# Gnnng/SVDFeature

Measured on AMD Instinct MI355X. Metric: training instances/sec (SGD updates/s), basicMF k=64, higher is better.
Workload: dtype f32; 1 GPU; basicMF synthetic 1000000x100000, 100000000 ratings, k=64 fp32 (BASELINE configs[1]); order=uniform random (file order preserved: result == sequential SGD), conflict_free_batches_per_pass=903, parallelism=1 GPU

## Files before the change

### svdfeature_amd/csrc/svdf_capi.cpp

```cpp
#include <svdfeature_amd.h>

#include <algorithm>
#include <cstdlib>
#include <cstring>
#include <new>
#include <vector>

#include "svdf_engine.h"
#include "svdf_kernels.h"

namespace svdf {
void rank_eval_metrics(long S, const int64_t *sec_ptr, const int *position, const int *ranked, const int *nan, int num_at, const int *at,
                       svdf_rank_metrics *out);
void set_error_mode(int m);
const char *last_error();
void note_error(const std::string &m);
}

struct svdf_trainer { svdf::Engine *e; };
struct svdf_dataset { svdf::Dataset *d; };
struct svdf_ranker { svdf::Ranker *r; };

#define SVDF_GUARD(retval, ...)                                 \
    try { __VA_ARGS__; }                                        \
// ... 219 lines not shown
    delete ds;
}
int svdf_train_dataset(svdf_trainer *t, svdf_dataset *ds) { SVDF_GUARD(-1, { t->e->train_dataset(ds->d); return 0; }) }
int svdf_predict_dataset(svdf_trainer *t, svdf_dataset *ds, float *out) { SVDF_GUARD(-1, { t->e->predict_dataset(ds->d, out); return 0; }) }
int64_t svdf_dataset_info(const svdf_dataset *ds, int what) {
    if (!ds || !ds->d) return -1;
    switch (what) {
    case 0: return ds->d->num_row;
    case 1: return ds->d->kind == 8 ? (int64_t)ds->d->wchild.size() : (int64_t)ds->d->sched.num_levels();
    case 2: return ds->d->sched.max_level_size;
    case 3: return ds->d->kind;
    case 4: return ds->d->algorithmic_bytes;
    case 5: return ds->d->num_units;
    case 6: return ds->d->num_simple_units;
    case 7: {
        uint64_t h = 1469598103934665603ull;
        auto mix = [&h](uint64_t v) { for (int b = 0; b < 8; b++) { h ^= (v >> (8 * b)) & 0xFFu; h *= 1099511628211ull; } };
        for (long v : ds->d->sched.level_ptr) mix((uint64_t)v);
        for (long v : ds->d->sched.level_mid) mix((uint64_t)v);
        for (int v : ds->d->sched.order) mix((uint64_t)(unsigned)v);
        return (int64_t)(h >> 1);
    }
    case 8: return ds->d->kind == 8 && !ds->d->wchild.empty() ? (int64_t)ds->d->wchild[0]->kind : -1;
    default: return -1;
    }
}

int svdf_item_delta_begin(svdf_trainer *t) { SVDF_GUARD(-1, { t->e->per_rank_api(); t->e->item_delta_begin(); return 0; }) }
void *svdf_item_delta_buffer(svdf_trainer *t, int64_t *count) { SVDF_GUARD(nullptr, { t->e->per_rank_api(); return t->e->item_delta_buffer(count); }) }
int svdf_item_delta_apply(svdf_trainer *t) { SVDF_GUARD(-1, { t->e->per_rank_api(); t->e->item_delta_apply(); return 0; }) }
int svdf_item_delta_export(svdf_trainer *t, float *dst) { SVDF_GUARD(-1, { t->e->per_rank_api(); t->e->item_delta_copy(dst, nullptr); return 0; }) }
int svdf_item_delta_import(svdf_trainer *t, const float *src) { SVDF_GUARD(-1, { t->e->per_rank_api(); t->e->item_delta_copy(nullptr, src); return 0; }) }

int svdf_item_delta_into(svdf_trainer *t, float *dst, int64_t *count) { SVDF_GUARD(-1, { t->e->per_rank_api(); t->e->item_delta_into(dst, count); return 0; }) }
int svdf_item_delta_pack(svdf_trainer *t, void *dst, int half, int64_t *count) { SVDF_GUARD(-1, { t->e->per_rank_api(); t->e->item_delta_pack(dst, half, count); return 0; }) }
int svdf_item_delta_unpack(svdf_trainer *t, const void *src, int half, int refresh_snapshot) {
    SVDF_GUARD(-1, { t->e->per_rank_api(); t->e->item_delta_unpack(src, half, refresh_snapshot); return 0; })
}
int svdf_item_delta_select(svdf_trainer *t, int part, int nparts) { SVDF_GUARD(-1, { t->e->per_rank_api(); t->e->item_delta_select(part, nparts); return 0; }) }
int svdf_item_delta_apply_from(svdf_trainer *t, const float *src) { SVDF_GUARD(-1, { t->e->per_rank_api(); t->e->item_delta_apply_from(src); return 0; }) }
int svdf_set_stream(svdf_trainer *t, void *hip_stream) { SVDF_GUARD(-1, { t->e->set_stream((hipStream_t)hip_stream); return 0; }) }

int64_t svdf_get_view(svdf_trainer *t, int which, float *out, int64_t capacity) { SVDF_GUARD(-1, { return t->e->get_view(which, out, capacity); }) }
int64_t svdf_set_view(svdf_trainer *t, int which, const float *in, int64_t count) { SVDF_GUARD(-1, { return t->e->set_view(which, in, count); }) }
int svdf_view_shape(svdf_trainer *t, int which, int *rows, int *cols) { SVDF_GUARD(-1, { t->e->view_shape(which, rows, cols); return 0; }) }
void *svdf_stream(svdf_trainer *t) { return (void *)t->e->stream(); }
// ... 91 lines not shown
```

### svdfeature_amd/csrc/svdf_config.cpp

```cpp
#include "svdf_engine.h"

#include <algorithm>
#include <chrono>
#include <cmath>
#include <cstdlib>
#include <cstring>
#include <memory>
#include <mutex>
#include <atomic>
#include <thread>

#include "svdf_kernels.h"
#include "svdf_internal.h"

namespace svdf {

void ParamSet::set_param(const char *name, const char *val) {
    if (!strncmp(name, prefix_a.c_str(), prefix_a.size())) name += prefix_a.size();
    else if (!strncmp(name, prefix_b.c_str(), prefix_b.size())) name += prefix_b.size();
    else return;
    if (!strcmp("bound", name)) {
        unsigned bd = (unsigned)atoi(val);
        check(bd > 0, "can't give 0 as bound");
        check(bound.empty() || bound.back() < bd, "bound must be given in order");
// ... 195 lines not shown
        check(value >= 0 && value <= 8 && value != 7, "groups_per_wave must be 0 (auto), 1 ... 6 or 8");
        groups_per_wave_ = (int)value;
        return 0;
    }
    if (!strcmp(name, "xcd_remap")) { xcd_remap_ = value != 0; params_dirty_ = true; return 0; }
    if (!strcmp(name, "fewrow_i16")) { check(value >= 0 && value <= 1, "fewrow_i16 must be 0 or 1"); fewrow_i16_ = (int)value; params_dirty_ = true; return 0; }
    if (!strcmp(name, "svdpp_helpers")) { check(value == 1 || value == 4 || value == 8 || value == 16, "svdpp_helpers must be 1, 4, 8 or 16"); svdpp_helpers_ = (int)value; params_dirty_ = true; return 0; }
    if (!strcmp(name, "basic_i8")) { check(value >= 0 && value <= 1, "basic_i8 must be 0 or 1"); basic_i8_ = (int)value; params_dirty_ = true; return 0; }
    if (!strcmp(name, "load_mode")) { check(value >= 0 && value <= 2, "load_mode must be 0, 1 or 2 (auto)"); load_mode_ = (int)value; params_dirty_ = true; return 0; }
    if (!strcmp(name, "store_mode")) { check(value >= 0 && value <= 2, "store_mode must be 0, 1 or 2"); store_mode_ = (int)value; params_dirty_ = true; return 0; }
    if (!strcmp(name, "sort_batches")) { check(value >= 0 && value <= 2, "sort_batches must be 0, 1 (by item) or 2 (by user)"); sort_batches_ = (int)value; return 0; }
    if (!strcmp(name, "async_flush")) { flush(); async_flush_ = value != 0; return 0; }
    if (!strcmp(name, "use_fused")) { use_fused_ = value != 0; return 0; }
    if (!strcmp(name, "device_schedule")) { device_sched_ = value != 0; return 0; }
    if (!strcmp(name, "device_rank")) { device_rank_ = value != 0; return 0; }
    if (!strcmp(name, "device_init")) { device_init_ = value != 0; return 0; }
    if (!strcmp(name, "device_window")) { device_window_ = value != 0; return 0; }
    if (!strcmp(name, "device_load")) { device_load_ = value != 0; return 0; }
    if (!strcmp(name, "runs_exec")) { check(value == 0 || value == 1, "runs_exec must be 0 or 1"); runs_exec_ = (int)value; return 0; }
    if (!strcmp(name, "runs_len")) { check(value >= 2 && value <= 7, "runs_len must be in 2 .. 7"); runs_len_ = (int)value; return 0; }
    if (!strcmp(name, "runs_sets")) { check(value >= 1 && value <= 2, "runs_sets must be 1 or 2"); runs_sets_ = (int)value; return 0; }
    if (!strcmp(name, "runs_block")) { check(value == 64 || value == 128 || value == 256, "runs_block must be 64, 128 or 256"); runs_block_ = (int)value; return 0; }
    if (!strcmp(name, "runs_min_rows")) { check(value >= 0, "runs_min_rows must not be negative"); runs_min_rows_ = value; return 0; }
    if (!strcmp(name, "pair_units")) { check(value == 0 || value == 1, "pair_units must be 0 or 1"); pair_units_ = (int)value; return 0; }
    if (!strcmp(name, "pair_unit_cap")) { check(value >= 1 && value <= 4096, "pair_unit_cap must be in 1 .. 4096"); pair_unit_cap_ = (int)value; return 0; }
    if (!strcmp(name, "pivot_exec")) { check(value == 0 || value == 1, "pivot_exec must be 0 or 1"); pivot_exec_ = (int)value; return 0; }
    if (!strcmp(name, "pivot_run")) { check(value >= 1 && value <= 65536, "pivot_run must be in 1 .. 65536"); pivot_run_ = (int)value; return 0; }
    if (!strcmp(name, "pivot_min")) { check(value >= 2, "pivot_min must be at least 2"); pivot_min_ = (int)value; return 0; }
    if (!strcmp(name, "ipc_spin_limit")) { ipc_set_spin_limit(value); return 0; }
    if (!strcmp(name, "chain_width")) { check(value >= 0, "chain_width must not be negative"); chain_width_ = value; return 0; }
    if (!strcmp(name, "device_init_margin_log2")) { check(value >= 8 && value <= 52, "device_init_margin_log2 must be in 8 .. 52"); device_init_margin_log2_ = (int)value; return 0; }
    if (!strcmp(name, "device_schedule_min")) { check(value >= 1, "device_schedule_min must be >= 1"); device_sched_min_ = value; return 0; }
    if (!strcmp(name, "use_simple_units")) { use_simple_units_ = value != 0; return 0; }
    if (!strcmp(name, "rows_without_feedback")) { rows_without_feedback_ = value != 0; return 0; }
    if (!strcmp(name, "fewrow_gslots")) { fewrow_gslots_ = value != 0; launch_version_++; return 0; }
    if (!strcmp(name, "staged_pool")) { check(value == 0 || value == 1, "staged_pool must be 0 or 1"); flush(); staged_pool_mode_ = (int)value; return 0; }
    if (!strcmp(name, "wunit_inplace")) { wunit_inplace_ = value != 0; return 0; }
    if (!strcmp(name, "wunit_defer_fb")) { wunit_defer_fb_ = value != 0; return 0; }
    if (!strcmp(name, "wunit_fast")) { check(value >= 0 && value <= 3, "wunit_fast must be 0, 1, 2 or 3"); wunit_fast_ = (int)value; return 0; }
    if (!strcmp(name, "window_per_target_child")) { check(value >= 1, "window_per_target_child must be positive"); wseq_per_target_child_ = (int)value; return 0; }
    if (!strcmp(name, "window_per_target_shared")) { check(value >= 1, "window_per_target_shared must be positive"); wseq_per_target_shared_ = (int)value; return 0; }
    if (!strcmp(name, "window_per_target_fb")) { check(value >= 1, "window_per_target_fb must be positive"); wseq_per_target_fb_ = (int)value; return 0; }
    if (!strcmp(name, "window_shared_sub")) { check(value >= 0 && value <= 4096, "window_shared_sub must be in 0 .. 4096"); wseq_shared_sub_ = (int)value; return 0; }
    if (!strcmp(name, "window_shared_max")) { check(value >= 1, "window_shared_max must be positive"); wseq_shared_max_ = (int)value; return 0; }
    if (!strcmp(name, "window_item_sub")) { check(value >= 0 && value <= 128, "window_item_sub must be in 0 .. 128"); wseq_item_sub_ = (int)value; return 0; }
    if (!strcmp(name, "window_item_max")) { check(value >= 1, "window_item_max must be positive"); wseq_item_max_ = (int)value; return 0; }
// ... 43 lines not shown
```

### svdfeature_amd/csrc/svdf_dataset.cpp

```cpp
#include "svdf_engine.h"

#include <algorithm>
#include <chrono>
#include <cmath>
#include <cstdlib>
#include <cstring>
#include <memory>
#include <mutex>
#include <atomic>
#include <thread>

#include "svdf_kernels.h"
#include "svdf_internal.h"

namespace svdf {

Dataset *Engine::dataset_from_blocks(long num_block, const int *extend_tag, const int64_t *fb_ptr, const unsigned *fb_index, const float *fb_value,
                                     const int64_t *block_row_ptr, const float *row_label, const int64_t *row_ptr, const unsigned *feat_index,
                                     const float *feat_value) {
    check(trainer_ready_, "dataset: init_trainer has not been called");
    need_device("dataset");
    check(user_group(), "svdfeature_amd: block datasets are for user-group (format_type 1) trainers");
    if (multi_ && !in_multi_scope()) {
        check(mp_.common_feedback_space == 0, "svdfeature_amd: amd:gpus > 1 needs a feedback space of its own (common_feedback_space = 0)");
// ... 568 lines not shown
    auto levels = [&](const char *what) { snprintf(buf, sizeof(buf), "exact, %ld conflict-free levels: %s", L, what); return std::string(buf); };
    switch (ds->kind) {
    case 0: return levels(chain_width_ > 0 ? "contract kernel k_basicmf / k_basicmf_slots, one (user, item) instance per lane group; narrow levels chained (k_basicmf_slots_chain)"
                                           : "contract kernel k_basicmf / k_basicmf_slots, one (user, item) instance per lane group");
    case 1: return levels("general sparse kernel k_general (any number of ids per row, side tables, lazy decay)");
    case 2: {
        const FusedSchedule S = ds->fused.view();
        if (fewrow_gslots_ && fewrow_fast_ && fewrow_gslots_applies(P, S, ds->fused.max_nu, ds->fused.max_ni, ds->fused.dense_slots))
            return levels("few-row kernel with global ids k_fewrow_gslots (neighbourhood shape)");
        return levels(fewrow_fast_ && fewrow_fast_applies(P, S) ? "few-row kernel k_fewrow_slots (<= 2 user + 2 item rows per instance: rank pairs, side ids); narrow levels chained"
                                                                 : "fused few-row kernel k_fused");
    }
    case 3: snprintf(buf, sizeof(buf), "exact, %ld conflict-free levels of user units: k_svdpp_wave (one wave per user, %ld of %ld units) + k_svdpp (general units)",
                     L, ds->num_simple_units, ds->num_units); return buf;
    case 4: return levels("multi-level implicit feedback units k_imfb");
    case 5: return "window data set (one window of the window-minibatch step, user side exact): k_window_users / k_window_items";
    case 6: return "amd:gpus handle: per-rank windows (svdf_multi.cpp)";
    case 7: return "window data set of user units: k_wunit_* (svdf_k_wunit.hip)";
    case 8: snprintf(buf, sizeof(buf), "window sequence (amd:step = minibatch / auto): %zu windows, each trained and applied in place%s%s; NOT the reference's sequential semantics (|dRMSE| <= 1e-4 contract)",
                     ds->wchild.size(), side_tables() ? ", feature_user / feature_item children as shared rows (general walk k_wunit_walk)" : "",
                     !ds->wchild.empty() && ds->wchild[0]->kind == 7 && !wunit_width_ok() ? ", user units of wide rows: the wide general walk k_wunit_walk<64, ., ., WideRow>, one wave per unit" : ""); return buf;
    case 9: snprintf(buf, sizeof(buf), "exact, %ld levels: hot rows walked as units (k_svdpp_wave on %s parameters, %ld units) + cold ratings through the contract kernel",
                     L, ds->pv_item_pivot ? "transposed" : "plain", ds->num_units); return buf;
    case 10: snprintf(buf, sizeof(buf), "exact, %ld levels of runs: k_basicmf_runs_soa (up to %d consecutive ratings of one item per lane group, the item's row in registers)", L, ds->rn_len); return buf;
    case 11: snprintf(buf, sizeof(buf), "exact, %ld levels of user-run units: k_pair_units (%ld units of up to %d consecutive pairs of one user, the user's row in registers)",
                      L, ds->num_units, pair_unit_cap_); return buf;
    default: return "unknown";
    }
}
void Engine::note_dataset(Dataset *ds) {
    if (!ds || host_only_ || is_peer_) return;
    const bool verbose = getenv("SVDF_VERBOSE") != nullptr, quiet = getenv("SVDF_QUIET") != nullptr;
    if (verbose && !quiet) fprintf(stderr, "[svdfeature_amd] data set of %ld rows -> %s\n", (long)ds->num_row, path_for(ds).c_str());
    if (step_auto_set_ || step_minibatch_set_ || multi_ || gpus_ != 1) return;
    if (!(ds->kind == 0 || ds->kind == 1 || ds->kind == 2 || ds->kind == 3 || ds->kind == 4 || ds->kind == 9 || ds->kind == 10 || ds->kind == 11) || ds->num_row <= 0) return;
    AutoDecision D;
    double unit_us = 4.5;
    auto_measures(ds, D.levels, unit_us, D.dag_ms, D.stream_ms, pivot_run_);
    guard_last_ = D;
    if (D.dag_ms <= 10.0 * D.stream_ms || D.dag_ms < 50.0) return;
    n_guard_warnings_++;
    if (quiet) return;
    const bool window_ok = ds->plain_rows ? wunit_config_ok(false) && window_rows_allowed() && (wseq_pair_sub_ == 0 || wunit_width_ok())
                                          : wunit_config_ok() && (ds->kind == 3 || ds->kind == 4 || basic_fast_path_allowed());
    fprintf(stderr, "[svdfeature_amd] default (exact) step: %ld rows in %ld conflict-free levels -- the data's dependency depth binds: about %.0f ms per pass "
                    "(%.2f M rows/s; levels x %.1f us) against %.1f ms if the rows streamed.  The exact pass keeps the reference's sequential result bit for bit; "
                    "%s\n",
// ... 235 lines not shown
```

### svdfeature_amd/csrc/svdf_engine.h

```cpp
#ifndef SVDF_ENGINE_H_
#define SVDF_ENGINE_H_

#include <hip/hip_runtime.h>

#include <condition_variable>
#include <cstdio>
#include <memory>
#include <mutex>
#include <stdexcept>
#include <thread>
#include <string>
#include <deque>
#include <functional>
#include <future>
#include <map>
#include <vector>

#include "svdf_types.h"

namespace svdf {

struct Error : std::runtime_error {
    explicit Error(const std::string &m) : std::runtime_error(m) {}
};
// ... 204 lines not shown
    size_t scan_tmp_bytes = 0;
    ~RankSource() { if (scan_tmp) (void)hipFree(scan_tmp); }
};
class Engine;
class Ranker;

struct Dataset {
    Engine *owner = nullptr;
    long num_row = 0;
    int kind = 0;
    DevBuf<WinUser> win_urec;
    DevBuf<int> win_slot, win_iptr, win_slot1;
    DevBuf<unsigned> win_item1;
    DevBuf<float> win_ival1;
    long win_item_lo = 0, win_item_hi = -1;
    DevBuf<long> d_level_ptr;
    bool d_level_ptr_ok = false;
    DevBuf<PairUnit> pu_units;
    DevBuf<unsigned> pu_lo, pu_hi;
    DevBuf<float> pu_vlo, pu_one;
    DevBuf<unsigned> rn_item, rn_user[8];
    DevBuf<float> rn_label[8];
    int rn_len = 0;
    std::vector<long> pv_unit_ptr;
    bool pv_item_pivot = false;
    long pv_cold = 0, pv_hot_rows = 0;
    int64_t chained_levels = 0;
    bool win_hot = false;
    long win_slots = 0;
    DevBuf<int> win_pos;
    bool win_has_pos = false;
    std::vector<long> wfirst;
    DevBuf<WinUnit> wu_units;
    DevBuf<WinSeg> wu_segs;
    DevBuf<int> wu_rptr, wu_tptr, wu_gptr;
    DevBuf<WinEnt> wu_ent, wu_fbent;
    DevBuf<WinTouched> wu_touched;
    long wu_ntouched = -1;
    DevBuf<WinFbRec> wu_fbrec;
    long wu_nseg = 0;
    bool wu_defer_fb = false;
    long wu_gslots = 0;
    int wu_estride = 0;
    bool wu_feedback = false;
    DevBuf<int> wu_uptr, wu_upos;
    DevBuf<WinEnt> wu_uent;
// ... 377 lines not shown
    long wseq_actual_csr(long W, long n, const int64_t *row_ptr, const unsigned *feat_index, const WseqCounts &C0, int shared_sub, int item_sub) const;
    bool wseq_hot_ok() const;
    long wseq_windows_hot(long n, const std::vector<long> &item_count) const;
    long wseq_windows_sub(long n, const std::vector<long> &item_count, int sub, int cap) const;
    void wseq_pair_check(const char *what) const;
    void wseq_sub_check(const char *what, const char *knob, const char *desc, const char *entry, const char *nrank, bool entry_only = false) const;
    std::vector<long> wseq_item_counts(long n, const unsigned *item, const unsigned *item1) const;
    Dataset *wseq_from_columns(long n, const unsigned *user, const unsigned *item, const unsigned *item1, const float *label, int sub, long W);
    double wseq_class_term(const std::vector<long> &cnt, int per) const;
    void wseq_count_targets(WseqCounts &C, long r0, long r1, const int64_t *row_ptr, const unsigned *feat_index) const;
    void wseq_adopt_window(Dataset *ds, const WUnitHost &H, long first);
    long wseq_windows_shared(long n, const std::vector<long> &plain, const std::vector<long> &child, int sub, int cap, int per_plain, int per_child) const;
    double wseq_max_ratio() const { return (double)wseq_per_target_ / (double)wseq_per_target_max_; }
    int wseq_per_target_ = 24;
    bool single_minibatch() const { return step_minibatch_set_ && gpus_ == 1 && !multi_ && !is_peer_; }
    int runs_exec_ = 1;
    int runs_len_ = 4;
    int runs_sets_ = 1, runs_block_ = 64;
    long runs_min_rows_ = 1 << 20;
    int64_t n_runs_passes_ = 0;
    bool runs_config_ok() const;
    Dataset *runs_dataset_from_triples(long n, const unsigned *user, const unsigned *item, const float *label);
    void runs_train(Dataset *ds);
    int pivot_exec_ = 1;
    int pivot_run_ = 256, pivot_run_long_ = 256;
    int pivot_min_ = 2048;
    int64_t n_pivot_passes_ = 0;
    int pair_units_ = 1, pair_unit_cap_ = 16;
    int64_t n_punit_passes_ = 0;
    bool punit_config_ok() const;
    Dataset *punit_dataset_from_pairs(long n, const unsigned *user, const unsigned *pos, const unsigned *neg);
    bool punit_build(long n, const unsigned *user, const unsigned *lo, const unsigned *hi, std::vector<PairUnit> &sorted, std::vector<long> &level_ptr) const;
    bool punit_flush(HostCSR &src);
    DevBuf<PairUnit> w_pu_units_;
    PairUnitSchedule punit_view(const Dataset *ds) const;
    void punit_train(Dataset *ds);
    void punit_predict(Dataset *ds, float *d_out);
    bool pivot_config_ok() const;
    Dataset *pivot_dataset_from_triples(long n, const unsigned *user, const unsigned *item, const float *label);
    void pivot_train(Dataset *ds);
    bool step_auto_set_ = false, auto_building_ = false;
    struct AutoDecision { int decided = 0; long levels = 0, windows = 0; double dag_ms = 0.0, stream_ms = 0.0; } auto_last_;
    bool auto_step_active() const { return step_auto_set_ && !auto_building_ && gpus_ == 1 && !multi_ && !is_peer_ && !host_only_; }
    Dataset *auto_step(Dataset *exact, bool window_ok, const std::function<Dataset *()> &build_window);
    static constexpr long AUTO_PROBE_ROWS = 2000000, AUTO_PROBE_MIN = 8000000;
    AutoDecision auto_probe_;
// ... 186 lines not shown
```

### svdfeature_amd/csrc/svdf_k_runs.hip

```cpp
#include "svdf_device.h"

namespace svdf {

__global__ __launch_bounds__(256) void k_runs_check(const unsigned *user, const unsigned *item, long n, unsigned nu, unsigned ni, unsigned *flag) {
    const long stride = (long)gridDim.x * blockDim.x;
    unsigned bad = 0u;
    for (long p = (long)blockIdx.x * blockDim.x + threadIdx.x; p < n; p += stride) {
        if (user[p] >= nu) bad |= 1u;
        if (item[p] >= ni) bad |= 2u;
    }
    if (bad) atomicOr(flag, bad);
}
__global__ __launch_bounds__(256) void k_runs_prev(const unsigned *keys, const unsigned *pos, long n, unsigned *prev) {
    const long stride = (long)gridDim.x * blockDim.x;
    for (long j = (long)blockIdx.x * blockDim.x + threadIdx.x; j < n; j += stride)
        prev[pos[j]] = (j > 0 && keys[j - 1] == keys[j]) ? pos[j - 1] : 0xFFFFFFFFu;
}
__global__ __launch_bounds__(256) void k_runs_form(const unsigned *ikeys, const unsigned *ipos, long n, unsigned num_item, const unsigned *prev, int R,
                                                   unsigned *head, unsigned *head_of, unsigned char *idx) {
    const long stride = (long)gridDim.x * blockDim.x;
    for (long it = (long)blockIdx.x * blockDim.x + threadIdx.x; it < (long)num_item; it += stride) {
        long lo = 0, hi = n;
        while (lo < hi) { const long mid = (lo + hi) >> 1; if (ikeys[mid] < (unsigned)it) lo = mid + 1; else hi = mid; }
        unsigned h = 0u;
// ... 35 lines not shown
}
void launch_runs_form(const unsigned *ikeys, const unsigned *ipos, long n, unsigned num_item, const unsigned *prev, int R, unsigned *head, unsigned *head_of,
                      unsigned char *idx, hipStream_t st) {
    if (n > 0 && num_item > 0) hipLaunchKernelGGL(k_runs_form, dim3(runs_grid((long)num_item)), dim3(256), 0, st, ikeys, ipos, n, num_item, prev, R, head, head_of, idx);
}
void launch_runs_fill(const unsigned *user, const unsigned *item, const float *label, long n, const unsigned *unit_at, const unsigned *head_of,
                      const unsigned char *idx, long nunit, unsigned *c_item, unsigned *c_user, float *c_label, hipStream_t st) {
    if (n > 0) hipLaunchKernelGGL(k_runs_fill, dim3(runs_grid(n)), dim3(256), 0, st, user, item, label, n, unit_at, head_of, idx, nunit, c_item, c_user, c_label);
}
__global__ __launch_bounds__(256) void k_runs_iota(unsigned *v, long n) {
    const long stride = (long)gridDim.x * blockDim.x;
    for (long j = (long)blockIdx.x * blockDim.x + threadIdx.x; j < n; j += stride) v[j] = (unsigned)j;
}
void launch_runs_iota(unsigned *v, long n, hipStream_t st) {
    if (n <= 0) return;
    long grid = (n + 255) / 256;
    if (grid > 16384) grid = 16384;
    hipLaunchKernelGGL(k_runs_iota, dim3((int)grid), dim3(256), 0, st, v, n);
}
void launch_runs_fill_u32(unsigned *v, long n, unsigned x, hipStream_t st) {
    if (n > 0) hipLaunchKernelGGL(k_runs_fill_u32, dim3(runs_grid(n)), dim3(256), 0, st, v, n, x);
}

template <int LANES, int V, int R, int G>
__global__ __launch_bounds__(256) void k_basicmf_runs_soa(const DevParams P, const RunSchedule S, long begin, long end) {
    constexpr int T = 16 / LANES;
    constexpr int IPS = 64 / LANES;
    constexpr int K = 4 * LANES * V;
    const int lane = threadIdx.x & 63;
    long tile = blockIdx.x;
    if (P.xcd_remap) tile = (long)(blockIdx.x & 7) * (gridDim.x >> 3) + (blockIdx.x >> 3);
    const long wave = tile * (blockDim.x >> 6) + (threadIdx.x >> 6);
    const int m = (lane & 15) / T;
    const int gslot = (lane >> 4) * T + (lane & (T - 1));
    const int pitch = P.pitch;
    const float dec_u1 = snap_to_one(1.0f - P.lr * P.wd_user), dec_i1 = snap_to_one(1.0f - P.lr * P.wd_item);
#pragma unroll 1
    for (int g = 0; g < G; g++) {
        const long w0 = begin + (wave * G + g) * IPS;
        if (w0 >= end) return;
        const long s = w0 + gslot;
        const bool live = s < end;
        const long sc = live ? s : w0;
        const unsigned ir = P.item_off + S.item[sc];
        unsigned ur[R];
        float label[R], bu[R];
        float4 p[R][V], q[V];
        int n = 0;
#pragma unroll
        for (int j = 0; j < R; j++) {
            const unsigned u = S.user[j][sc];
            label[j] = S.label[j][sc];
            const bool on = live && u != (unsigned)SLOT_ABSENT;
            ur[j] = P.user_off + (on ? u : 0u);
            if (on) n = j + 1;
        }
#pragma unroll
        for (int v = 0; v < V; v++) q[v] = live ? load_row_nt<K / 4>(P.W, ir, pitch, m + v * LANES, K) : f4zero();
        float bi = live ? P.bias[ir] : 0.0f;
#pragma unroll
        for (int j = 0; j < R; j++) {
#pragma unroll
            for (int v = 0; v < V; v++) p[j][v] = f4zero();
            bu[j] = 0.0f;
            if (j < n) {
#pragma unroll
                for (int v = 0; v < V; v++) p[j][v] = load_row_nt<K / 4>(P.W, ur[j], pitch, m + v * LANES, K);
                bu[j] = P.bias[ur[j]];
            }
        }
#pragma unroll
        for (int j = 0; j < R; j++) asm volatile("" :: "v"(p[j][0].x), "v"(p[j][V - 1].x), "v"(bu[j]));
#pragma unroll
        for (int j = 0; j < R; j++) {
            if (!__any(j < n)) break;
            double bs = 0.0;
            bs += (double)(1.0f * bu[j]); bs += 0.0;
            bs += 0.0;
            bs += (double)(1.0f * bi);
            double sum = (double)P.base_score + bs;
            float4 tu[V], ti[V];
#pragma unroll
            for (int v = 0; v < V; v++) { tu[v] = f4zero(); ti[v] = f4zero(); axpy4(tu[v], p[j][v], 1.0f); axpy4(ti[v], q[v], 1.0f); }
            sum += (double)dot_slots<LANES, V>(tu, ti, m, lane);
            const float pred = (float)sum;
            const float err = (label[j] - pred) * 1.0f;
            const float su = P.lr * err * 1.0f;
            const float si = P.lr * err * 1.0f;
            float nbu = bu[j] + su, nbi = bi + si;
            nbu = nbu * (1.0f - P.lr * P.wd_user_bias);
            nbi = nbi * (1.0f - P.lr * P.wd_item_bias);
            const bool act = j < n;
#pragma unroll
            for (int v = 0; v < V; v++) {
                float4 wu = p[j][v], wi = q[v];
                axpy4(wu, ti[v], su);
                axpy4(wi, tu[v], si);
                wu.x = wu.x * dec_u1; wu.y = wu.y * dec_u1; wu.z = wu.z * dec_u1; wu.w = wu.w * dec_u1;
                wi.x = wi.x * dec_i1; wi.y = wi.y * dec_i1; wi.z = wi.z * dec_i1; wi.w = wi.w * dec_i1;
                if (act) {
                    store_row<K / 4>(P.W, ur[j], pitch, m + v * LANES, K, wu);
                    q[v] = wi;
                }
            }
            if (act) {
                P.bias[ur[j]] = nbu;
                bi = nbi;
            }
        }
        if (live) {
#pragma unroll
            for (int v = 0; v < V; v++) store_row<K / 4>(P.W, ir, pitch, m + v * LANES, K, q[v]);
            P.bias[ir] = bi;
        }
    }
}
bool basicmf_runs_soa_applies(const DevParams &P) {
    return P.basic_i8 && P.active_type == ACT_LINEAR && P.reg_method == 0 && P.no_user_bias == 0 && P.user_nonnegative == 0 && P.u_rng.n == 0 && P.i_rng.n == 0 &&
           P.store_mode == 0 && (P.k == 64 || P.k == 128);
}
void launch_basicmf_runs_soa(const DevParams &P, const RunSchedule &S, long begin, long end, int R, int G, int block_threads, hipStream_t st) {
    if (end <= begin) return;
    if (G < 1) G = 1;
    if (block_threads != 64 && block_threads != 128 && block_threads != 256) block_threads = 64;
    const int per_wave = P.k == 128 ? 4 : 8;
    const long per_block = (long)(block_threads / 64) * G * per_wave;
    int grid = (int)((end - begin + per_block - 1) / per_block);
    if (P.xcd_remap) grid = (grid + 7) & ~7;
#define RUNS_LAUNCH(L_, R_, G_) hipLaunchKernelGGL((k_basicmf_runs_soa<L_, 2, R_, G_>), dim3(grid), dim3(block_threads), 0, st, P, S, begin, end)
#define RUNS_BY_R(L_)                                                                                                          \
    if (R == 2) { if (G >= 2) RUNS_LAUNCH(L_, 2, 2); else RUNS_LAUNCH(L_, 2, 1); }       \
    else if (R == 4) { if (G >= 2) RUNS_LAUNCH(L_, 4, 2); else RUNS_LAUNCH(L_, 4, 1); }                                       \
    else { if (G >= 2) RUNS_LAUNCH(L_, 7, 2); else RUNS_LAUNCH(L_, 7, 1); }
    if (P.k == 128) { RUNS_BY_R(16) } else { RUNS_BY_R(8) }
#undef RUNS_BY_R
#undef RUNS_LAUNCH
}

}
```

### svdfeature_amd/csrc/svdf_kernels.h

```cpp
#ifndef SVDF_KERNELS_H_
#define SVDF_KERNELS_H_

#include <hip/hip_runtime.h>

#include <type_traits>
#include <vector>

#include "svdf_types.h"

namespace svdf {

int lanes_per_instance(int k);
int max_supported_factor();
int max_fast_path_factor();

void launch_basicmf(const DevParams &P, const BasicSchedule &S, long begin, long end, int groups_per_wave, int block_threads, hipStream_t st);
bool launch_basicmf_chain(const DevParams &P, const BasicSchedule &S, const long *d_level_ptr, long l0, long l1, hipStream_t st);
void launch_fused(const DevParams &P, const FusedSchedule &S, int max_nu, int max_ni, long begin, long end, int groups_per_wave,
                  int block_threads, hipStream_t st);
bool fewrow_fast_applies(const DevParams &P, const FusedSchedule &S);
bool launch_fewrow_chain(const DevParams &P, const FusedSchedule &S, int max_nu, int max_ni, const long *d_level_ptr, long l0, long l1, hipStream_t st);
bool fewrow_gslots_applies(const DevParams &P, const FusedSchedule &S, int max_nu, int max_ni, bool dense_slots);
void launch_fewrow_gslots(const DevParams &P, const FusedSchedule &S, long begin, long end, hipStream_t st);
void launch_fewrow_fast(const DevParams &P, const FusedSchedule &S, int max_nu, int max_ni, long begin, long end, int block_threads, hipStream_t st);
// ... 63 lines not shown
struct RselSecs { unsigned K1[RANK_TILE]; };
long rank_tile_minima(long n);
bool rank_tile_select_applies(long n, long cap, long K1max);
void launch_rank_tile_select(long n, long cap, int nsec, const unsigned *keys, const unsigned *wmin, const RselSecs &Ks, unsigned *out, long out_stride,
                             const unsigned *flag, hipStream_t st);
void launch_rank_select_tile(long n, long cap, int nsec, const unsigned *keys, const RselSecs &Ks, unsigned *work, unsigned *ck, unsigned *cv, unsigned *out,
                             long out_stride, unsigned *flag, hipStream_t st);
void launch_rank_positions(long n, const float *score, const signed char *tag, const int *pos_item, int npos, int *greater, int *ties, hipStream_t st);
long rank_select_work_words();
long rank_select_cap();
void launch_rank_select(long n, const unsigned *keys, const unsigned *vals, unsigned K1, unsigned *work, unsigned *ck, unsigned *cv, unsigned *out,
                        const unsigned *flag, hipStream_t st);
long device_exclusive_scan_u32(const unsigned *in, unsigned *out, long n, void **tmp, size_t *tmp_bytes, hipStream_t st);
void launch_runs_check(const unsigned *user, const unsigned *item, long n, unsigned nu, unsigned ni, unsigned *flag, hipStream_t st);
void launch_runs_prev(const unsigned *keys, const unsigned *pos, long n, unsigned *prev, hipStream_t st);
void launch_runs_form(const unsigned *ikeys, const unsigned *ipos, long n, unsigned num_item, const unsigned *prev, int R, unsigned *head, unsigned *head_of,
                      unsigned char *idx, hipStream_t st);
void launch_runs_fill(const unsigned *user, const unsigned *item, const float *label, long n, const unsigned *unit_at, const unsigned *head_of,
                      const unsigned char *idx, long nunit, unsigned *c_item, unsigned *c_user, float *c_label, hipStream_t st);
bool pair_units_applies(const DevParams &P);
void launch_pair_units(const DevParams &P, const PairUnitSchedule &S, long begin, long end, float *out, hipStream_t st);
void launch_runs_iota(unsigned *v, long n, hipStream_t st);
void launch_runs_fill_u32(unsigned *v, long n, unsigned x, hipStream_t st);
bool basicmf_runs_soa_applies(const DevParams &P);
void launch_basicmf_runs_soa(const DevParams &P, const RunSchedule &S, long begin, long end, int R, int G, int block_threads, hipStream_t st);
void device_sort_pairs_u32(unsigned *keys_in, unsigned *keys_out, unsigned *vals_in, unsigned *vals_out, long n, void **tmp, size_t *tmp_bytes, hipStream_t st);
int sqerr_partials_grid(long n);
void launch_sqerr_partials(const float *pred, const float *label, long n, float scale, double *partials, hipStream_t st);
struct RankSourceDev {
    long num_block, num_row;
    const long *block_row_ptr;
    const float *label, *uval, *ival;
    const unsigned *uidx, *iidx;
};
struct SamplerParams { float pos_lowerb, neg_upperb; int sample_num, sample_max; };
struct PairColumns { float *label, *uval, *v0, *v1; unsigned *uidx, *i0, *i1; };
struct RankRowsDev {
    long num_block, num_row;
    const long *block_row_ptr;
    const float *label;
    const int *row_ptr;
    const unsigned *index;
    const float *value;
};
struct GSamplerParams { float pos_lowerb, neg_upperb, gap; int sample_num, sample_max, method, method_raw, pointwise; };
void launch_gsample_counts(const RankRowsDev &S, const GSamplerParams &sp, int *scratch, long *draws, long *pairs, hipStream_t st);
// ... 118 lines not shown
```

### svdfeature_amd/csrc/svdf_runs.cpp

```cpp
#include <algorithm>
#include <cstring>
#include <memory>

#include "svdf_engine.h"
#include "svdf_kernels.h"
#include "svdf_internal.h"

namespace svdf {

bool Engine::runs_config_ok() const {
    return runs_exec_ != 0 && !host_only_ && device_sched_ && !user_group() && basic_fast_path_allowed() && mtype_.extend_type == 0 && mtype_.active_type == ACT_LINEAR &&
           tp_.reg_method == 0 && mp_.user_nonnegative == 0 && mp_.no_user_bias == 0 && u_param_.bound.empty() && i_param_.bound.empty() && (mp_.num_factor == 64 || mp_.num_factor == 128) &&
           basic_i8_ != 0 && store_mode_ == 0;
}

Dataset *Engine::runs_dataset_from_triples(long n, const unsigned *user, const unsigned *item, const float *label) {
    if (!runs_config_ok() || n < runs_min_rows_ || n >= 0x7FFFFFF0L) return nullptr;
    const int RF = std::max(2, std::min(7, runs_len_));
    const int R = RF <= 2 ? 2 : (RF <= 4 ? 4 : 7);
    const unsigned NU = (unsigned)mp_.num_user, NI = (unsigned)mp_.num_item;
    std::unique_ptr<Dataset> ds(new Dataset());
    adopt(ds.get());
    ds->kind = 10; ds->num_row = n; ds->rn_len = R;
    ds->user.upload(user, (size_t)n, stream_);
// ... 27 lines not shown
    const long nunit = device_exclusive_scan_u32(head.p, unit_at.p, n, &tmp, &tmp_bytes, stream_);
    HIPCHECK(hipGetLastError());
    c_item.reserve((size_t)nunit); c_user.reserve((size_t)R * (size_t)nunit); c_label.reserve((size_t)R * (size_t)nunit);
    launch_runs_fill_u32(c_user.p, (long)R * nunit, (unsigned)SLOT_ABSENT, stream_);
    HIPCHECK(hipMemsetAsync(c_label.p, 0, (size_t)R * (size_t)nunit * sizeof(float), stream_));
    launch_runs_fill(ds->user.p, ds->item.p, ds->label.p, n, unit_at.p, head_of.p, idx.p, nunit, c_item.p, c_user.p, c_label.p, stream_);
    HIPCHECK(hipGetLastError());
    HIPCHECK(hipStreamSynchronize(stream_));
    ka.release(); kb.release(); va.release(); vb.release(); prev.release(); head.release(); head_of.release(); unit_at.release(); idx.release();
    const unsigned *res[SVDF_SCHED_MAX_SLOTS];
    unsigned off[SVDF_SCHED_MAX_SLOTS], limit[SVDF_SCHED_MAX_SLOTS];
    const char *msg[SVDF_SCHED_MAX_SLOTS];
    res[0] = c_item.p; off[0] = NU; limit[0] = NI; msg[0] = "item feature index exceed bound";
    std::vector<DUCol> du{DUCol{c_item.p, &ds->rn_item}};
    std::vector<DFCol> df;
    for (int j = 0; j < R; j++) {
        res[1 + j] = c_user.p + (size_t)j * (size_t)nunit; off[1 + j] = 0u; limit[1 + j] = NU; msg[1 + j] = "user feature index exceed bound";
        du.push_back(DUCol{c_user.p + (size_t)j * (size_t)nunit, &ds->rn_user[j]});
        df.push_back(DFCol{c_label.p + (size_t)j * (size_t)nunit, &ds->rn_label[j]});
    }
    schedule_device_columns(ds.get(), nunit, 1 + R, res, off, limit, msg, sort_batches_ == 1 ? c_item.p : nullptr, NI, du, df);
    ds->num_units = nunit;
    ds->algorithmic_bytes = n * (8L * mp_.num_factor * 2 + 8 * 2 + 16 + 8 * 2);
    return ds.release();
}

void Engine::runs_train(Dataset *ds) {
    const DevParams &P = params();
    RunSchedule S;
    memset(&S, 0, sizeof(S));
    S.item = ds->rn_item.p;
    for (int j = 0; j < ds->rn_len; j++) { S.user[j] = ds->rn_user[j].p; S.label[j] = ds->rn_label[j].p; }
    const Schedule &sc = ds->sched;
    for (size_t l = 0; l < sc.num_levels(); l++) launch_basicmf_runs_soa(P, S, sc.level_ptr[l], sc.level_ptr[l + 1], ds->rn_len, runs_sets_, runs_block_, stream_);
    HIPCHECK(hipGetLastError());
    n_launches_ += (int64_t)sc.num_levels();
    n_batches_ += (int64_t)sc.num_levels();
    n_runs_passes_++;
}

}
```

### svdfeature_amd/csrc/svdf_types.h

```cpp
#ifndef SVDF_TYPES_H_
#define SVDF_TYPES_H_

#include <stdint.h>

namespace svdf {

struct TypeParam {
    uint8_t format_type, active_type, extend_type, variant_type;
};
static_assert(sizeof(TypeParam) == 4, "SVDTypeParam is 4 bytes");

struct ModelParam {
    int num_user, num_item, num_factor, num_global;
    float u_init_sigma, i_init_sigma, base_score;
    int no_user_bias, num_ufeedback;
    float ufeedback_init_sigma;
    int num_randinit_ufactor, num_randinit_ifactor;
    int common_latent_space, user_nonnegative, common_feedback_space, extend_flag, item_nonnegative;
    int reserved[247];
};
static_assert(sizeof(ModelParam) == 1056, "SVDModelParam is 1056 bytes on disk");

struct TrainParam {
    float learning_rate;
// ... 50 lines not shown
    int small_blocks;
    int basic_i8;
    int load_mode;
    float lr, wd_user, wd_item, wd_user_bias, wd_item_bias, wd_global;
    int reg_method, reg_global;
    unsigned num_regfree_global;
    float scale_lr_ufeedback, wd_ufeedback, wd_ufeedback_bias;
    DevRanges u_rng, i_rng, g_rng;
    DevSideTable feat_user, feat_item;
};

struct BasicSchedule {
    const unsigned *user;
    const unsigned *item;
    const float *label;
    const float *uval;
    const float *ival;
};

struct RunSchedule {
    const unsigned *item;
    const unsigned *user[8];
    const float *label[8];
};

struct PairUnit { unsigned user; int begin; int count; int pad; };
struct PairUnitSchedule {
    const PairUnit *units;
    const unsigned *lo, *hi;
    const float *vlo;
};

struct FusedSchedule {
    const float *label;
    const unsigned *uidx[2];
    const float *uval[2];
    const unsigned *iidx[2];
    const float *ival[2];
    const int *gptr;
    const unsigned *gidx;
    const float *gval;
    const unsigned *gsi[4];
    const float *gsv[4];
};
enum { SLOT_ABSENT = 0xFFFFFFFFu };

struct DevCSR {
// ... 100 lines not shown
```

Before: 5.939 billion instances/s.

## Stage runs kernel operands in schedule-ordered slots, handing rows between consecutive runs

Adds an operand-staging mode, on by default, for the basicMF runs kernel. Each (run, operand) pair gets its own slot in schedule order, and a one-time device sort builds next-occurrence links. Each run then reads its user and item rows and biases contiguously from the staging buffer and writes updated rows into the slot of that row's next use, or back to W at its last use. A stage-in kernel copies each row's initial value into its first slot before every pass. The aim is to turn random gathers from W into streaming reads. The cost is a large extra device buffer sized by ratings × pitch, plus a per-pass stage-in, and the mode falls back to plain W when memory is short.

Measured after the change: 6.217 billion instances/s (median of 6 runs). +4.7%, better.

```diff
diff --git a/svdfeature_amd/csrc/svdf_capi.cpp b/svdfeature_amd/csrc/svdf_capi.cpp
--- a/svdfeature_amd/csrc/svdf_capi.cpp
+++ b/svdfeature_amd/csrc/svdf_capi.cpp
@@ -265,6 +265,8 @@
         return (int64_t)(h >> 1);
     }
     case 8: return ds->d->kind == 8 && !ds->d->wchild.empty() ? (int64_t)ds->d->wchild[0]->kind : -1;
+    case 9: return ds->d->rn_stage_state;
+    case 10: return ds->d->rn_stage_bytes;
     default: return -1;
     }
 }
diff --git a/svdfeature_amd/csrc/svdf_config.cpp b/svdfeature_amd/csrc/svdf_config.cpp
--- a/svdfeature_amd/csrc/svdf_config.cpp
+++ b/svdfeature_amd/csrc/svdf_config.cpp
@@ -241,6 +241,8 @@
     if (!strcmp(name, "runs_sets")) { check(value >= 1 && value <= 2, "runs_sets must be 1 or 2"); runs_sets_ = (int)value; return 0; }
     if (!strcmp(name, "runs_block")) { check(value == 64 || value == 128 || value == 256, "runs_block must be 64, 128 or 256"); runs_block_ = (int)value; return 0; }
     if (!strcmp(name, "runs_min_rows")) { check(value >= 0, "runs_min_rows must not be negative"); runs_min_rows_ = value; return 0; }
+    if (!strcmp(name, "runs_stage")) { check(value == 0 || value == 1, "runs_stage must be 0 or 1"); runs_stage_ = (int)value; return 0; }
+    if (!strcmp(name, "runs_stage_max_mb")) { check(value >= -1, "runs_stage_max_mb must be -1 (no cap) or a size in MB"); runs_stage_max_mb_ = value; return 0; }
     if (!strcmp(name, "pair_units")) { check(value == 0 || value == 1, "pair_units must be 0 or 1"); pair_units_ = (int)value; return 0; }
     if (!strcmp(name, "pair_unit_cap")) { check(value >= 1 && value <= 4096, "pair_unit_cap must be in 1 .. 4096"); pair_unit_cap_ = (int)value; return 0; }
     if (!strcmp(name, "pivot_exec")) { check(value == 0 || value == 1, "pivot_exec must be 0 or 1"); pivot_exec_ = (int)value; return 0; }
diff --git a/svdfeature_amd/csrc/svdf_dataset.cpp b/svdfeature_amd/csrc/svdf_dataset.cpp
--- a/svdfeature_amd/csrc/svdf_dataset.cpp
+++ b/svdfeature_amd/csrc/svdf_dataset.cpp
@@ -614,7 +614,13 @@
                      !ds->wchild.empty() && ds->wchild[0]->kind == 7 && !wunit_width_ok() ? ", user units of wide rows: the wide general walk k_wunit_walk<64, ., ., WideRow>, one wave per unit" : ""); return buf;
     case 9: snprintf(buf, sizeof(buf), "exact, %ld levels: hot rows walked as units (k_svdpp_wave on %s parameters, %ld units) + cold ratings through the contract kernel",
                      L, ds->pv_item_pivot ? "transposed" : "plain", ds->num_units); return buf;
-    case 10: snprintf(buf, sizeof(buf), "exact, %ld levels of runs: k_basicmf_runs_soa (up to %d consecutive ratings of one item per lane group, the item's row in registers)", L, ds->rn_len); return buf;
+    case 10: {
+        char st[96] = "rows in W";
+        if (runs_staged(ds)) snprintf(st, sizeof(st), "rows handed from run to run through staging slots (runs_stage, %.1f MB)", (double)ds->rn_stage_bytes / 1048576.0);
+        else if (ds->rn_stage_state == 2) snprintf(st, sizeof(st), "rows in W (operand staging refused)");
+        snprintf(buf, sizeof(buf), "exact, %ld levels of runs: k_basicmf_runs_soa (up to %d consecutive ratings of one item per lane group, the item's row in registers); %s", L, ds->rn_len, st);
+        return buf;
+    }
     case 11: snprintf(buf, sizeof(buf), "exact, %ld levels of user-run units: k_pair_units (%ld units of up to %d consecutive pairs of one user, the user's row in registers)",
                       L, ds->num_units, pair_unit_cap_); return buf;
     default: return "unknown";
diff --git a/svdfeature_amd/csrc/svdf_engine.h b/svdfeature_amd/csrc/svdf_engine.h
--- a/svdfeature_amd/csrc/svdf_engine.h
+++ b/svdfeature_amd/csrc/svdf_engine.h
@@ -250,6 +250,11 @@
     DevBuf<unsigned> rn_item, rn_user[8];
     DevBuf<float> rn_label[8];
     int rn_len = 0;
+    DevBuf<float> rn_stage_row, rn_stage_bias;
+    DevBuf<unsigned> rn_dst, rn_first;
+    int rn_stage_state = 0;
+    unsigned rn_stage_row0 = 0;
+    int64_t rn_stage_bytes = 0;
     std::vector<long> pv_unit_ptr;
     bool pv_item_pivot = false;
     long pv_cold = 0, pv_hot_rows = 0;
@@ -673,6 +678,10 @@
     bool runs_config_ok() const;
     Dataset *runs_dataset_from_triples(long n, const unsigned *user, const unsigned *item, const float *label);
     void runs_train(Dataset *ds);
+    int runs_stage_ = 1;
+    long runs_stage_max_mb_ = -1;
+    void runs_stage_build(Dataset *ds);
+    bool runs_staged(const Dataset *ds) const { return runs_stage_ != 0 && ds->rn_stage_state == 1 && ds->rn_stage_row0 == user_off_; }
     int pivot_exec_ = 1;
     int pivot_run_ = 256, pivot_run_long_ = 256;
     int pivot_min_ = 2048;
diff --git a/svdfeature_amd/csrc/svdf_k_runs.hip b/svdfeature_amd/csrc/svdf_k_runs.hip
--- a/svdfeature_amd/csrc/svdf_k_runs.hip
+++ b/svdfeature_amd/csrc/svdf_k_runs.hip
@@ -81,7 +81,63 @@
     if (n > 0) hipLaunchKernelGGL(k_runs_fill_u32, dim3(runs_grid(n)), dim3(256), 0, st, v, n, x);
 }
 
-template <int LANES, int V, int R, int G>
+__global__ __launch_bounds__(256) void k_runs_inverse(const int *order, long nunit, unsigned *pos_of) {
+    const long stride = (long)gridDim.x * blockDim.x;
+    for (long s = (long)blockIdx.x * blockDim.x + threadIdx.x; s < nunit; s += stride) pos_of[order[s]] = (unsigned)s;
+}
+__global__ __launch_bounds__(256) void k_runs_operands(const RunSchedule S, const unsigned *pos_of, long nunit, int R, unsigned num_user, unsigned *keys, unsigned *vals) {
+    const long stride = (long)gridDim.x * blockDim.x, m = nunit * (1 + R);
+    for (long t = (long)blockIdx.x * blockDim.x + threadIdx.x; t < m; t += stride) {
+        const long un = t / (1 + R);
+        const int j = (int)(t - un * (1 + R));
+        const unsigned s = pos_of[un];
+        const unsigned id = j == 0 ? num_user + S.item[s] : S.user[j - 1][s];
+        keys[t] = (j > 0 && id == (unsigned)SLOT_ABSENT) ? 0xFFFFFFFFu : id;
+        vals[t] = (unsigned)((long)j * nunit + s);
+    }
+}
+__global__ __launch_bounds__(256) void k_runs_links(const unsigned *keys, const unsigned *vals, long m, unsigned row0, unsigned *dst, unsigned *first) {
+    const long stride = (long)gridDim.x * blockDim.x;
+    for (long t = (long)blockIdx.x * blockDim.x + threadIdx.x; t < m; t += stride) {
+        const unsigned key = keys[t], slot = vals[t];
+        if (key == 0xFFFFFFFFu) { dst[slot] = (unsigned)SLOT_ABSENT; continue; }
+        dst[slot] = (t + 1 < m && keys[t + 1] == key) ? vals[t + 1] : ((unsigned)RUNS_HOME | (row0 + key));
+        if (t == 0 || keys[t - 1] != key) first[key] = slot;
+    }
+}
+void launch_runs_stage_links(const RunSchedule &S, const int *order, long nunit, int R, unsigned num_user, unsigned row0, unsigned *pos_of, unsigned *ka, unsigned *kb,
+                             unsigned *va, unsigned *vb, void **tmp, size_t *tmp_bytes, unsigned *dst, unsigned *first, long nrow, hipStream_t st) {
+    if (nunit <= 0) return;
+    const long m = nunit * (1 + R);
+    hipLaunchKernelGGL(k_runs_inverse, dim3(runs_grid(nunit)), dim3(256), 0, st, order, nunit, pos_of);
+    hipLaunchKernelGGL(k_runs_operands, dim3(runs_grid(m)), dim3(256), 0, st, S, pos_of, nunit, R, num_user, ka, va);
+    device_sort_pairs_u32(ka, kb, va, vb, m, tmp, tmp_bytes, st);
+    launch_runs_fill_u32(first, nrow, (unsigned)SLOT_ABSENT, st);
+    hipLaunchKernelGGL(k_runs_links, dim3(runs_grid(m)), dim3(256), 0, st, kb, vb, m, row0, dst, first);
+}
+template <int LPR>
+__global__ __launch_bounds__(256) void k_runs_stage_in(const DevParams P, const unsigned *first, long nrow, unsigned row0, float *stage_row, float *stage_bias) {
+    const int L = threadIdx.x % LPR;
+    const long per = 256 / LPR, stride = (long)gridDim.x * per;
+    for (long r = (long)blockIdx.x * per + threadIdx.x / LPR; r < nrow; r += stride) {
+        const unsigned slot = first[r];
+        if (slot == (unsigned)SLOT_ABSENT) continue;
+        store_row<LPR>(stage_row, slot, P.pitch, L, P.k, load_row_nt<LPR>(P.W, (size_t)row0 + (size_t)r, P.pitch, L, P.k));
+        if (L == 0) stage_bias[slot] = P.bias[(size_t)row0 + (size_t)r];
+    }
+}
+void launch_runs_stage_in(const DevParams &P, const unsigned *first, long nrow, unsigned row0, float *stage_row, float *stage_bias, hipStream_t st) {
+    if (nrow <= 0) return;
+    const long per = P.k == 128 ? 8 : 16;
+    long grid = (nrow + per - 1) / per;
+    if (grid > 16384) grid = 16384;
+    if (P.k == 128) hipLaunchKernelGGL(k_runs_stage_in<32>, dim3((int)grid), dim3(256), 0, st, P, first, nrow, row0, stage_row, stage_bias);
+    else hipLaunchKernelGGL(k_runs_stage_in<16>, dim3((int)grid), dim3(256), 0, st, P, first, nrow, row0, stage_row, stage_bias);
+}
+
+__device__ __forceinline__ unsigned load_u32_nt(const unsigned *p) { return __builtin_nontemporal_load(p); }
+__device__ __forceinline__ float load_f32_nt(const float *p) { return __builtin_nontemporal_load(p); }
+template <int LANES, int V, int R, int G, bool STAGED>
 __global__ __launch_bounds__(256) void k_basicmf_runs_soa(const DevParams P, const RunSchedule S, long begin, long end) {
     constexpr int T = 16 / LANES;
     constexpr int IPS = 64 / LANES;
@@ -101,31 +157,59 @@
         const long s = w0 + gslot;
         const bool live = s < end;
         const long sc = live ? s : w0;
-        const unsigned ir = P.item_off + S.item[sc];
-        unsigned ur[R];
-        float label[R], bu[R];
+        unsigned ir, ur[R];
+        float label[R], bu[R], bi;
         float4 p[R][V], q[V];
         int n = 0;
-#pragma unroll
-        for (int j = 0; j < R; j++) {
-            const unsigned u = S.user[j][sc];
-            label[j] = S.label[j][sc];
-            const bool on = live && u != (unsigned)SLOT_ABSENT;
-            ur[j] = P.user_off + (on ? u : 0u);
-            if (on) n = j + 1;
-        }
-#pragma unroll
-        for (int v = 0; v < V; v++) q[v] = live ? load_row_nt<K / 4>(P.W, ir, pitch, m + v * LANES, K) : f4zero();
-        float bi = live ? P.bias[ir] : 0.0f;
-#pragma unroll
-        for (int j = 0; j < R; j++) {
-#pragma unroll
-            for (int v = 0; v < V; v++) p[j][v] = f4zero();
-            bu[j] = 0.0f;
-            if (j < n) {
-#pragma unroll
-                for (int v = 0; v < V; v++) p[j][v] = load_row_nt<K / 4>(P.W, ur[j], pitch, m + v * LANES, K);
-                bu[j] = P.bias[ur[j]];
+        if constexpr (!STAGED) {
+            ir = P.item_off + S.item[sc];
+#pragma unroll
+            for (int j = 0; j < R; j++) {
+                const unsigned u = S.user[j][sc];
+                label[j] = S.label[j][sc];
+                const bool on = live && u != (unsigned)SLOT_ABSENT;
+                ur[j] = P.user_off + (on ? u : 0u);
+                if (on) n = j + 1;
+            }
+#pragma unroll
+            for (int v = 0; v < V; v++) q[v] = live ? load_row_nt<K / 4>(P.W, ir, pitch, m + v * LANES, K) : f4zero();
+            bi = live ? P.bias[ir] : 0.0f;
+#pragma unroll
+            for (int j = 0; j < R; j++) {
+#pragma unroll
+                for (int v = 0; v < V; v++) p[j][v] = f4zero();
+                bu[j] = 0.0f;
+                if (j < n) {
+#pragma unroll
+                    for (int v = 0; v < V; v++) p[j][v] = load_row_nt<K / 4>(P.W, ur[j], pitch, m + v * LANES, K);
+                    bu[j] = P.bias[ur[j]];
+                }
+            }
+        } else {
+            const size_t nun = (size_t)S.nunit, at0 = (size_t)sc;
+            ir = load_u32_nt(S.dst + at0);
+#pragma unroll
+            for (int j = 0; j < R; j++) {
+                ur[j] = load_u32_nt(S.dst + (size_t)(1 + j) * nun + at0);
+                label[j] = S.label[j][sc];
+            }
+#pragma unroll
+            for (int j = 0; j < R; j++)
+                if (live && ur[j] != (unsigned)SLOT_ABSENT) n = j + 1;
+#pragma unroll
+            for (int v = 0; v < V; v++) q[v] = live ? load_row_nt<K / 4>(S.stage_row, at0, pitch, m + v * LANES, K) : f4zero();
+            bi = live ? load_f32_nt(S.stage_bias + at0) : 0.0f;
+#pragma unroll
+            for (int j = 0; j < R; j++) {
+#pragma unroll
+                for (int v = 0; v < V; v++) p[j][v] = f4zero();
+                bu[j] = 0.0f;
+                if (j < n) {
+                    const size_t at = (size_t)(1 + j) * nun + at0;
+#pragma unroll
+                    for (int v = 0; v < V; v++) p[j][v] = load_row_nt<K / 4>(S.stage_row, at, pitch, m + v * LANES, K);
+                    bu[j] = load_f32_nt(S.stage_bias + at);
+                }
             }
         }
 #pragma unroll
@@ -150,6 +234,13 @@
             nbu = nbu * (1.0f - P.lr * P.wd_user_bias);
             nbi = nbi * (1.0f - P.lr * P.wd_item_bias);
             const bool act = j < n;
+            float *wb = P.W, *bb = P.bias;
+            size_t wr = ur[j];
+            if constexpr (STAGED) {
+                const bool home = (ur[j] & (unsigned)RUNS_HOME) != 0u;
+                wb = home ? P.W : S.stage_row; bb = home ? P.bias : S.stage_bias;
+                wr = ur[j] & ~(unsigned)RUNS_HOME;
+            }
 #pragma unroll
             for (int v = 0; v < V; v++) {
                 float4 wu = p[j][v], wi = q[v];
@@ -158,19 +249,26 @@
                 wu.x = wu.x * dec_u1; wu.y = wu.y * dec_u1; wu.z = wu.z * dec_u1; wu.w = wu.w * dec_u1;
                 wi.x = wi.x * dec_i1; wi.y = wi.y * dec_i1; wi.z = wi.z * dec_i1; wi.w = wi.w * dec_i1;
                 if (act) {
-                    store_row<K / 4>(P.W, ur[j], pitch, m + v * LANES, K, wu);
+                    store_row<K / 4>(wb, wr, pitch, m + v * LANES, K, wu);
                     q[v] = wi;
                 }
             }
             if (act) {
-                P.bias[ur[j]] = nbu;
+                bb[wr] = nbu;
                 bi = nbi;
             }
         }
         if (live) {
-#pragma unroll
-            for (int v = 0; v < V; v++) store_row<K / 4>(P.W, ir, pitch, m + v * LANES, K, q[v]);
-            P.bias[ir] = bi;
+            float *wb = P.W, *bb = P.bias;
+            size_t wr = ir;
+            if constexpr (STAGED) {
+                const bool home = (ir & (unsigned)RUNS_HOME) != 0u;
+                wb = home ? P.W : S.stage_row; bb = home ? P.bias : S.stage_bias;
+                wr = ir & ~(unsigned)RUNS_HOME;
+            }
+#pragma unroll
+            for (int v = 0; v < V; v++) store_row<K / 4>(wb, wr, pitch, m + v * LANES, K, q[v]);
+            bb[wr] = bi;
         }
     }
 }
@@ -186,7 +284,11 @@
     const long per_block = (long)(block_threads / 64) * G * per_wave;
     int grid = (int)((end - begin + per_block - 1) / per_block);
     if (P.xcd_remap) grid = (grid + 7) & ~7;
-#define RUNS_LAUNCH(L_, R_, G_) hipLaunchKernelGGL((k_basicmf_runs_soa<L_, 2, R_, G_>), dim3(grid), dim3(block_threads), 0, st, P, S, begin, end)
+#define RUNS_LAUNCH(L_, R_, G_)                                                                                                                          \
+    do {                                                                                                                                                \
+        if (S.dst) hipLaunchKernelGGL((k_basicmf_runs_soa<L_, 2, R_, G_, true>), dim3(grid), dim3(block_threads), 0, st, P, S, begin, end);              \
+        else hipLaunchKernelGGL((k_basicmf_runs_soa<L_, 2, R_, G_, false>), dim3(grid), dim3(block_threads), 0, st, P, S, begin, end);                   \
+    } while (0)
 #define RUNS_BY_R(L_)                                                                                                          \
     if (R == 2) { if (G >= 2) RUNS_LAUNCH(L_, 2, 2); else RUNS_LAUNCH(L_, 2, 1); }       \
     else if (R == 4) { if (G >= 2) RUNS_LAUNCH(L_, 4, 2); else RUNS_LAUNCH(L_, 4, 1); }                                       \
diff --git a/svdfeature_amd/csrc/svdf_kernels.h b/svdfeature_amd/csrc/svdf_kernels.h
--- a/svdfeature_amd/csrc/svdf_kernels.h
+++ b/svdfeature_amd/csrc/svdf_kernels.h
@@ -109,6 +109,9 @@
 void launch_pair_units(const DevParams &P, const PairUnitSchedule &S, long begin, long end, float *out, hipStream_t st);
 void launch_runs_iota(unsigned *v, long n, hipStream_t st);
 void launch_runs_fill_u32(unsigned *v, long n, unsigned x, hipStream_t st);
+void launch_runs_stage_links(const RunSchedule &S, const int *order, long nunit, int R, unsigned num_user, unsigned row0, unsigned *pos_of, unsigned *ka, unsigned *kb,
+                             unsigned *va, unsigned *vb, void **tmp, size_t *tmp_bytes, unsigned *dst, unsigned *first, long nrow, hipStream_t st);
+void launch_runs_stage_in(const DevParams &P, const unsigned *first, long nrow, unsigned row0, float *stage_row, float *stage_bias, hipStream_t st);
 bool basicmf_runs_soa_applies(const DevParams &P);
 void launch_basicmf_runs_soa(const DevParams &P, const RunSchedule &S, long begin, long end, int R, int G, int block_threads, hipStream_t st);
 void device_sort_pairs_u32(unsigned *keys_in, unsigned *keys_out, unsigned *vals_in, unsigned *vals_out, long n, void **tmp, size_t *tmp_bytes, hipStream_t st);
diff --git a/svdfeature_amd/csrc/svdf_runs.cpp b/svdfeature_amd/csrc/svdf_runs.cpp
--- a/svdfeature_amd/csrc/svdf_runs.cpp
+++ b/svdfeature_amd/csrc/svdf_runs.cpp
@@ -73,7 +73,65 @@
     schedule_device_columns(ds.get(), nunit, 1 + R, res, off, limit, msg, sort_batches_ == 1 ? c_item.p : nullptr, NI, du, df);
     ds->num_units = nunit;
     ds->algorithmic_bytes = n * (8L * mp_.num_factor * 2 + 8 * 2 + 16 + 8 * 2);
+    if (runs_stage_) runs_stage_build(ds.get());
     return ds.release();
+}
+
+namespace {
+template <typename T>
+bool try_reserve(DevBuf<T> &b, size_t n) {
+    b.release();
+    if (hipMalloc((void **)&b.p, (n ? n : 1) * sizeof(T)) != hipSuccess) { (void)hipGetLastError(); b.p = nullptr; return false; }
+    b.cap = n ? n : 1;
+    return true;
+}
+}
+void Engine::runs_stage_build(Dataset *ds) {
+    ds->rn_stage_state = 2;
+    ds->rn_stage_bytes = 0;
+    const long nunit = ds->num_units, nrow = (long)mp_.num_user + (long)mp_.num_item;
+    const int R = ds->rn_len;
+    const long m = (long)(1 + R) * nunit;
+    if (nunit <= 0) return;
+    const int64_t bytes = (int64_t)m * ((int64_t)pitch_ * 4 + 8) + (int64_t)nrow * 4;
+    auto refuse = [&](const char *why) {
+        ds->rn_stage_row.release(); ds->rn_stage_bias.release(); ds->rn_dst.release(); ds->rn_first.release();
+        if (!getenv("SVDF_QUIET"))
+            fprintf(stderr, "[svdfeature_amd] data set of %ld rows: no operand staging (%.1f MB: %s); its runs keep reading and writing W\n", (long)ds->num_row, (double)bytes / 1048576.0, why);
+    };
+    if (item_off_ != user_off_ + (unsigned)mp_.num_user || n_uiset_ >= 0x7FFFFFFFL) { refuse("W_user and W_item are not adjacent in W"); return; }
+    if (m >= 0x7FFFFFFFL) { refuse("more than 2^31 slots"); return; }
+    if (runs_stage_max_mb_ >= 0 && bytes > (int64_t)runs_stage_max_mb_ * 1048576) { refuse("above runs_stage_max_mb"); return; }
+    size_t free_b = 0, total_b = 0;
+    if (hipMemGetInfo(&free_b, &total_b) != hipSuccess) { (void)hipGetLastError(); refuse("hipMemGetInfo failed"); return; }
+    if ((uint64_t)bytes > (uint64_t)free_b / 2) { refuse("more than half of the free device memory"); return; }
+    if (!try_reserve(ds->rn_stage_row, (size_t)m * (size_t)pitch_) || !try_reserve(ds->rn_stage_bias, (size_t)m) || !try_reserve(ds->rn_dst, (size_t)m) ||
+        !try_reserve(ds->rn_first, (size_t)nrow)) { refuse("hipMalloc failed"); return; }
+    void *tmp = nullptr;
+    size_t tmp_bytes = 0;
+    struct FreeTmp { void *&p; ~FreeTmp() { if (p) (void)hipFree(p); } } free_tmp{tmp};
+    try {
+        DevBuf<unsigned> pos_of, ka, kb, va, vb;
+        if (!try_reserve(pos_of, (size_t)nunit) || !try_reserve(ka, (size_t)m) || !try_reserve(kb, (size_t)m) || !try_reserve(va, (size_t)m) || !try_reserve(vb, (size_t)m)) {
+            refuse("hipMalloc failed");
+            return;
+        }
+        RunSchedule S;
+        memset(&S, 0, sizeof(S));
+        S.item = ds->rn_item.p;
+        for (int j = 0; j < R; j++) S.user[j] = ds->rn_user[j].p;
+        launch_runs_stage_links(S, ds->order_dev.p, nunit, R, (unsigned)mp_.num_user, user_off_, pos_of.p, ka.p, kb.p, va.p, vb.p, &tmp, &tmp_bytes, ds->rn_dst.p,
+                                ds->rn_first.p, nrow, stream_);
+        HIPCHECK(hipGetLastError());
+        HIPCHECK(hipStreamSynchronize(stream_));
+    } catch (const std::exception &ex) {
+        (void)hipGetLastError();
+        refuse(ex.what());
+        return;
+    }
+    ds->rn_stage_state = 1;
+    ds->rn_stage_row0 = user_off_;
+    ds->rn_stage_bytes = bytes;
 }
 
 void Engine::runs_train(Dataset *ds) {
@@ -83,6 +141,12 @@
     S.item = ds->rn_item.p;
     for (int j = 0; j < ds->rn_len; j++) { S.user[j] = ds->rn_user[j].p; S.label[j] = ds->rn_label[j].p; }
     const Schedule &sc = ds->sched;
+    if (runs_stage_ && ds->rn_stage_state == 0) runs_stage_build(ds);
+    if (runs_staged(ds)) {
+        S.dst = ds->rn_dst.p; S.stage_row = ds->rn_stage_row.p; S.stage_bias = ds->rn_stage_bias.p; S.nunit = ds->num_units;
+        launch_runs_stage_in(P, ds->rn_first.p, (long)mp_.num_user + (long)mp_.num_item, user_off_, S.stage_row, S.stage_bias, stream_);
+        n_launches_++;
+    }
     for (size_t l = 0; l < sc.num_levels(); l++) launch_basicmf_runs_soa(P, S, sc.level_ptr[l], sc.level_ptr[l + 1], ds->rn_len, runs_sets_, runs_block_, stream_);
     HIPCHECK(hipGetLastError());
     n_launches_ += (int64_t)sc.num_levels();
diff --git a/svdfeature_amd/csrc/svdf_types.h b/svdfeature_amd/csrc/svdf_types.h
--- a/svdfeature_amd/csrc/svdf_types.h
+++ b/svdfeature_amd/csrc/svdf_types.h
@@ -96,7 +96,12 @@
     const unsigned *item;
     const unsigned *user[8];
     const float *label[8];
-};
+    const unsigned *dst;
+    float *stage_row;
+    float *stage_bias;
+    long nunit;
+};
+enum : unsigned { RUNS_HOME = 0x80000000u };
 
 struct PairUnit { unsigned user; int begin; int count; int pad; };
 struct PairUnitSchedule {
```
